# EricSteinberger/PokerRL

Hardware: AMD Instinct MI355X
Metric: CFR+ node-updates/sec on FHP public tree (higher is better)
Workload: dtype f32

## Files before the change

### include/pokerrl_hip.h

```cpp
#ifndef POKERRL_HIP_H
#define POKERRL_HIP_H

#include <stdint.h>

#ifdef __cplusplus
extern "C" {
#endif

#define PRL_MAX_BET_SIZES 96

#define PRL_OK 0
#define PRL_ERR_ARG (-1)
#define PRL_ERR_NO_DEVICE (-2)
#define PRL_ERR_HIP (-3)
#define PRL_ERR_UNSUPPORTED (-4)
#define PRL_ERR_OOM (-5)
#define PRL_ERR_STATE (-6)

typedef struct PrlRules {
    int32_t n_hole_cards;
    int32_t n_ranks;
    int32_t n_suits;
    int32_t n_cards;
    int32_t range_size;
// ... 223 lines not shown
    PRL_SF_STRAT_F64 = 4,
    PRL_SF_REGRET = 5,
    PRL_SF_AVG = 6,
    PRL_SF_AVG_F64 = 7,
    PRL_SF_AVG_SUM = 8,
    PRL_SF_BR_IDX = 9,
    PRL_SF_EXPL_HISTORY = 10,
    PRL_SF_ITER = 11,
    PRL_SF_CONSTANTS = 12,
    PRL_SF_BYTES_ALLOCATED = 13,
    PRL_SF_ENGINE = 14,
    PRL_SF_GRAPH_REPLAY = 15,
    PRL_SF_EXCHANGES = 17,
    PRL_SF_VMM_RANGES = 18,
    PRL_SF_AVG_PAIRS = 19,
    PRL_SF_EXPLICIT_STRATEGY = 16
};
int32_t prl_solver_get(prl_solver_t* solver, int32_t field, void* out);
int32_t prl_solver_set_strategy_device(prl_solver_t* solver, const prl_tree_t* tree, const float* d_probs, int32_t n_actions);
int32_t prl_solver_get_cols(prl_solver_t* solver, int32_t field, int64_t col_begin, int64_t n_cols, void* out);

int32_t prl_lbr_checkdown_equity(const PrlRules* rules, const int8_t* board_dealt, int32_t n_dealt, const int8_t* lbr_hand,
                                 const float* ranges, int32_t n_q, float* out_wp);
int32_t prl_lbr_checkdown_equity_batch(const PrlRules* rules, int32_t n_req, const int8_t* boards_dealt , const int32_t* n_dealt,
                                       const int8_t* lbr_hands , const float* ranges ,
                                       const int32_t* n_q, int32_t q_stride, float* out_wp );

int32_t prl_lbr_batch_run(const PrlGame* lbr_game, const PrlGame* agent_game, const PrlRules* rules, int32_t n_envs, int32_t agent_seat,
                          int32_t check_to_round, int32_t agent_kind, uint32_t agent_seed, uint32_t episode_base, double reward_scalar,
                          double ev_normalizer, const int8_t* cards, float* out_winnings, uint64_t* out_stats4, float* out_device_ms);
// ... 35 lines not shown
```

### pokerrl_amd/_native.py

```python
import ctypes
import os

import numpy as np

_HERE = os.path.dirname(os.path.abspath(__file__))
EXCHANGE_FN = ctypes.CFUNCTYPE(ctypes.c_int32, ctypes.c_void_p, ctypes.c_void_p, ctypes.c_void_p, ctypes.c_uint64)
LIB_PATH = os.environ.get("POKERRL_AMD_LIB", os.path.join(_HERE, "lib", "libpokerrl_hip.so"))

PRL_MAX_BET_SIZES = 96


class NativeError(RuntimeError):
    status = None


ERR_ARG, ERR_NO_DEVICE, ERR_HIP, ERR_UNSUPPORTED, ERR_OOM, ERR_STATE = -1, -2, -3, -4, -5, -6


class PrlRules(ctypes.Structure):
    _fields_ = [
        ("n_hole_cards", ctypes.c_int32), ("n_ranks", ctypes.c_int32), ("n_suits", ctypes.c_int32),
        ("n_cards", ctypes.c_int32), ("range_size", ctypes.c_int32), ("n_rounds", ctypes.c_int32),
        ("board_cards_in_round", ctypes.c_int32 * 4), ("n_board_cards", ctypes.c_int32),
        ("btn_first_postflop", ctypes.c_int32), ("rank_rule", ctypes.c_int32),
# ... 511 lines not shown
        check(self._L.prl_tree_obs_stats(self._h, _ptr(out)), self._L)
        return dict(state_bytes=int(out[0]), states_ms=float(out[1]), obs_ms=float(out[2]), obs_bytes=int(out[3]))

    def __del__(self):
        try:
            if self._h:
                self._L.prl_tree_destroy(self._h)
                self._h = None
        except Exception:
            pass


OBS_VANILLA, OBS_HISTORY, OBS_FLAT_HU_LIMIT = 0, 1, 2

SF = dict(reach=0, ev=1, ev_br=2, strategy=3, strat_f64=4, regret=5, avg=6, avg_f64=7, avg_sum=8, br_idx=9,
          expl_history=10, iter=11, constants=12, bytes_allocated=13, engine=14, graph_replay=15, explicit_strategy=16, exchanges=17, vmm_ranges=18, avg_pairs=19)
VARIANTS = {"vanilla": 0, "plus": 1, "linear": 2}
ENGINES = {"auto": 0, "levels": 1, "fused": 2}


class NativeSolver:

    def __init__(self, tree, variant, delay=0, engine="auto", _lib=None, shard=None, avg_dtype="f64", place=None, probe_iters=4, board_mult=None,
                 symmetrize=False):
        self._L = _lib or tree._L
        self.placement_ms, self.placement_chosen = None, None
        if _lib is None and self._L is lib():
            require_device()
        self.tree = tree
        self._h = ctypes.c_void_p()
        v = VARIANTS[variant] if isinstance(variant, str) else int(variant)
# ... 226 lines not shown
        finally:
            for n in names:
                qs[n].put(None)
            for t in th:
                t.join()
        return {n: h.hexdigest() for n, h in hs.items()}

    def get(self, name):
        n, c, R = self.n_nodes, self.n_cols, self.R
        shape, dtype = {
            "reach": ((n, 2, R), np.float32), "ev": ((n, 2, R), np.float32), "ev_br": ((n, 2, R), np.float32),
            "strategy": ((c, R), np.float64), "strat_f64": ((n,), np.uint8), "regret": ((c, R), np.float32),
            "avg": ((c, R), np.float64), "avg_f64": ((n,), np.uint8), "avg_sum": ((c, R), np.float32),
            "br_idx": ((n, R), np.int32), "constants": ((2,), np.float32), "bytes_allocated": ((1,), np.int64),
            "explicit_strategy": ((1,), np.int32), "exchanges": ((1,), np.int64), "vmm_ranges": ((2,), np.int64),
            "avg_pairs": ((1,), np.int64),
        }.get(name, (None, None))
        if name == "expl_history":
            shape, dtype = (self.iter + 1, 2), np.float32
        out = np.zeros(shape, dtype)
        self._call("prl_solver_get", SF[name], _ptr(out))
        return out
```

### pokerrl_amd/csrc/prl_fhp.h

```cpp
#pragma once
#include "prl_defs.h"
#include "prl_solver_types.h"
#include "prl_tree.h"

enum { PRL_SRC_REGRET = 0, PRL_SRC_UNIFORM64 = 1, PRL_SRC_ARR64 = 2, PRL_SRC_ARR32 = 3,
       PRL_SRC_STRAT32 = 4 ,
       PRL_SRC_AVGF32 = 5  };
enum { PRL_FHP_UPDATE0 = 0, PRL_FHP_UPDATE1 = 1, PRL_FHP_EVAL = 2, PRL_FHP_UPDATE0_EVAL = 3, PRL_FHP_UPDATE0_BR = 4, PRL_FHP_UPDATE1_EVAL1 = 5,
       PRL_FHP_EVAL0 = 6 };
constexpr bool prl_fhp_runs_seat(int mode, int p) {
    return mode == PRL_FHP_EVAL || mode == PRL_FHP_UPDATE0_EVAL ? true
         : (mode == PRL_FHP_UPDATE1 || mode == PRL_FHP_UPDATE1_EVAL1) ? p == 1 : p == 0;
}
constexpr bool prl_fhp_updates(int mode, int p) {
    return p == 0 ? (mode == PRL_FHP_UPDATE0 || mode == PRL_FHP_UPDATE0_EVAL || mode == PRL_FHP_UPDATE0_BR)
                  : (mode == PRL_FHP_UPDATE1 || mode == PRL_FHP_UPDATE1_EVAL1);
}
constexpr bool prl_fhp_with_br(int mode) { return mode >= PRL_FHP_EVAL; }
constexpr int prl_fhp_out_width(int mode) {
    return mode == PRL_FHP_UPDATE1_EVAL1 ? 3
         : (prl_fhp_runs_seat(mode, 0) && prl_fhp_runs_seat(mode, 1) ? 2 : 1) * (prl_fhp_with_br(mode) ? 2 : 1);
}

#define PRL_FHP_MAX_NODES 40
// ... 134 lines not shown
    int32_t np;
    int32_t variant, iter;
    int32_t max_grid;
    int32_t shape;
    int32_t n_cols_board, n_dec;
    int32_t dec_nch[PRL_FHP_MAX_DEC], dec_col0[PRL_FHP_MAX_DEC];
    float chance_prob, eq_const;
    float pot[PRL_FHP_MAX_NODES];
    const float* chance_reach;
    const float* board_w;
    float* regret;
    double* avg;
    float* avg32;
    int32_t avg_mode;
    double m_old, m_new;
    int32_t avg_pair;
    double m_old_prev, m_new_prev;
    float* avg_sum;
    int32_t avgsum_mask, avgsum_iter[2];
    int32_t block_sum;
    int32_t exp;
    int32_t no_steady;
    const double* strat_arr;
    float* board_out;
    const int16_t* plan_pp;
    const uint32_t* plan_clx;
    unsigned long long* timing;
};

int prl_fhp_match_shape(const PrlFlatTree& t, int* chance_node, int* first_board_node, int* col_base, float* pots );

int prl_launch_fhp_pass(const PrlFhpParams& prm, int mode, int src0, int src1, void* stream);
void prl_launch_fhp_strategy_from_regret(const PrlFhpParams& prm, double* out_region, void* stream);
void prl_launch_fhp_avg_from_sum(const PrlFhpParams& prm, void* stream);
void prl_launch_fhp_symmetrize(const float* in, int n_vec, int R, const int32_t* class_of, const int32_t* class_start, const int32_t* class_hands, float* out, void* stream);
void prl_launch_fhp_expand(const PrlFhpParams& prm, const void* region, int elem, int b0, int nb, const void* fill_by_col, const void* blocked_src,
                           void* dst, void* stream);
void prl_launch_fhp_compact(const PrlFhpParams& prm, const void* src, int elem, int b0, int nb, void* region, void* blocked_dst, void* stream);
#define PRL_FHP_NBLOCKED (1326 - 1081)
void prl_launch_fhp_chance_sum(const float* d_board_vals, int n_boards, int W, float* d_scratch, float* d_dest, void* stream);
int prl_fhp_units_at_level(int n_boards, int level);
void prl_launch_fhp_chance_partial(const float* d_board_vals, int n_boards, int level, int W, float* d_scratch, float* d_units, void* stream);
void prl_launch_fhp_chance_partial_from_blocks(const float* d_blocks, int n_blk, int level, int W, float* d_units, void* stream);
void prl_launch_fhp_chance_finish(const float* d_units, int n_units, int level, int W, float* d_scratch, float* d_dest, void* stream);
void prl_launch_fhp_compact_gathered(const float* d_in, int world, int n_which, int n_units, int W, float* d_out, void* stream);
```

### pokerrl_amd/csrc/prl_fhp_kernels.hip

```cpp
#include <type_traits>

#include "prl_device.h"
#include "prl_fhp.h"
#include "prl_kernels.h"


#if defined(PRL_EMU)
#define FHP_LB(t, w)
#else
#define FHP_LB(t, w) __launch_bounds__(t, w)
#endif

#define FHP_THREADS 768
#define FHP_SLOTS 2
#define FHP_LAUNCH_BOUNDS FHP_LB(768, 3)
#define FHP_SPEC PrlFhpSpec15
namespace fhp_shape15 {
#include "prl_fhp_pass.inc"
}
#undef FHP_SPEC
#define FHP_SPEC PrlFhpSpec9
namespace fhp_shape9 {
#include "prl_fhp_pass.inc"
}
#undef FHP_SPEC
#if !defined(PRL_FHP_NO_SHAPE21)
#define FHP_SPEC PrlFhpSpec21
namespace fhp_shape21 {
#include "prl_fhp_pass.inc"
}
#undef FHP_SPEC
#endif
#undef FHP_THREADS
#undef FHP_SLOTS
#undef FHP_LAUNCH_BOUNDS

const PrlFhpShapeDesc& prl_fhp_shape_desc(int shape_id) {
    static_assert(PrlFhpDerive<PrlFhpSpec15>::MAX_A <= PRL_FHP_BOARD_MAX_ACTIONS && PrlFhpDerive<PrlFhpSpec9>::MAX_A <= PRL_FHP_BOARD_MAX_ACTIONS &&
                      PrlFhpDerive<PrlFhpSpec21>::MAX_A <= PRL_FHP_BOARD_MAX_ACTIONS,
                  "the board pass and the readers of PrlFhpParams::dec_nch hold PRL_FHP_BOARD_MAX_ACTIONS actions per node");
    static const PrlFhpShapeDesc d[PRL_FHP_N_SHAPES] = {prl_fhp_describe<PrlFhpDerive<PrlFhpSpec15>>(), prl_fhp_describe<PrlFhpDerive<PrlFhpSpec9>>(),
                                                        prl_fhp_describe<PrlFhpDerive<PrlFhpSpec21>>()};
    return d[shape_id];
}

bool prl_fhp_shape_compiled(int shape_id) {
#if !defined(PRL_FHP_NO_SHAPE21)
    return shape_id >= 0 && shape_id < PRL_FHP_N_SHAPES;
#else
    return shape_id == PRL_FHP_SHAPE_15 || shape_id == PRL_FHP_SHAPE_9;
// ... 215 lines not shown
```

### pokerrl_amd/csrc/prl_fhp_pass.inc

```
#ifndef FHP_NPAD
#define FHP_NPAD 1088
#define FHP_NLIVE 1081
#define FHP_NCARDS 52
#define FHP_R 1326
#define FHP_NP PRL_FHP_NP
#define FHP_NSHOW (PrlFhpShape::N_SHOW)
#define FHP_NFOLD (PrlFhpShape::N_FOLD)
#define FHP_NVEC (PrlFhpShape::N_SHOW + PrlFhpShape::N_FOLD)
#endif
typedef PrlFhpDerive<FHP_SPEC> PrlFhpShape;
#if defined(FHP_EXPERIMENT)
#define FHP_EXP(c, bit) (((c).prm->exp & (bit)) != 0)
#define FHP_AVG_PIPELINED(c) true
#define FHP_TERMINAL_CACHE(c) true
#else
#define FHP_EXP(c, bit) false
#define FHP_AVG_PIPELINED(c) true
#define FHP_TERMINAL_CACHE(c) true
#endif
static_assert(PrlFhpShape::subtree_size(0) == PrlFhpShape::N_NODES, "the spec is one DFS pre-order tree");
static_assert(FHP_NP == FHP_NPAD && FHP_NP == PRL_PP_NPAD && FHP_R == PRL_PP_R && FHP_SLOTS == 2, "sorted storage: a column holds the padded sorted domain, a lane two positions");

#include "prl_fhp_div.inc"
struct FhpV { FhpF v; };
// ... 146 lines not shown

PRL_DEV PRL_INLINE FhpLds fhp_lds() {
    FhpLds L;
    float* f = (float*)prl_smem();
    L.y = f; f += FHP_NVEC * FHP_NPAD;
    L.K = f; f += 2 * FHP_NSHOW * FHP_NPAD;
    L.Tc = f; f += FHP_NFOLD * 64;
    L.Tt = f; f += 16;
    L.acc = f; f += FHP_ACC_WORDS;
    L.pf_rg = f; f += FHP_RG_IN_LDS ? FHP_PF_RG_WORDS : 0;
    L.pf_clx = (uint32_t*)f; f += FHP_PF_AREA(PRL_CLX_WORDS);
    L.pf_pp = (uint32_t*)f; f += FHP_PF_AREA(FHP_PP_WORDS);
    return L;
}

constexpr bool fhp_steady_plus(int steady) { return steady == 1 || steady == 4 || steady == 5 || steady == 6; }
template <int STEADY>
struct FhpCtxT {
    static constexpr bool own_after_b(int src_opp) { return src_opp == PRL_SRC_REGRET && !fhp_steady_plus(STEADY); }
    PRL_DEV PRL_INLINE int variant() const {
        if constexpr (fhp_steady_plus(STEADY)) return PRL_CFR_PLUS;
        else if constexpr (STEADY == 2) return PRL_CFR_LINEAR;
        else if constexpr (STEADY == 3) return PRL_CFR_VANILLA;
        else return variant_;
    }
    PRL_DEV PRL_INLINE bool first_iteration() const { if constexpr (STEADY != 0) return false; else return iter == 0; }
    PRL_DEV PRL_INLINE int avg_mode() const {
        if constexpr (STEADY == 1 || STEADY == 4 || STEADY == 6) return 2;
        else if constexpr (STEADY != 0) return 0;
        else return prm->avg_pair == PRL_FHP_AVG_DEFERRED ? 0 : prm->avg_mode;
    }
    PRL_DEV PRL_INLINE bool avg_catch_up() const { if constexpr (STEADY == 6) return true; else if constexpr (STEADY != 0) return false; else return prm->avg_pair == PRL_FHP_AVG_CATCH_UP; }
    PRL_DEV PRL_INLINE int avgsum_mask() const { if constexpr (fhp_steady_plus(STEADY)) return 0; else return prm->avgsum_mask; }
    PRL_DEV PRL_INLINE bool avg32() const { if constexpr (STEADY == 4) return true; else if constexpr (STEADY != 0) return false; else return prm->avg32 != nullptr; }
    FhpLds L;
    int wave;
    uint32_t pf_lds;
    uint32_t rec0, rec1;
    int p0;
    int gsm1[FHP_SLOTS];
    int gem1[FHP_SLOTS];
    bool live[FHP_SLOTS];
    int c1[FHP_SLOTS], c2[FHP_SLOTS];
    int sh[FHP_SLOTS];
    bool active;
    bool valid;
    float eq_const;
// ... 213 lines not shown
        if (lane == LAST_LANES - 1) L.Tt[v] = pj;
    };
    for (int v = wave; v < FHP_NVEC; v += n_waves) {
        if (v < 2 * FHP_NPAIRS) range_prefix(std::integral_constant<int, 2>(), v);
        else range_prefix(std::integral_constant<int, 1>(), v);
    }
    prl_dma_wait();
    FHP_SYNC(c, 3);
}

constexpr bool fhp_is_dec_of(int P, int n) { return PrlFhpShape::kind(n) == PRL_NODE_DECISION && PrlFhpShape::actor(n) == P; }
constexpr bool fhp_completes_before(int a, int b) {
    if (a > b) return a < b + PrlFhpShape::subtree_size(b);
    return !(b < a + PrlFhpShape::subtree_size(a));
}
constexpr int fhp_completion_rank(int P, int n) {
    int r = 0;
    for (int m = 0; m < PrlFhpShape::N_NODES; ++m)
        if (m != n && fhp_is_dec_of(P, m) && fhp_completes_before(m, n)) ++r;
    return r;
}
constexpr int fhp_node_of_rank(int P, int r) {
    for (int m = 0; m < PrlFhpShape::N_NODES; ++m)
        if (fhp_is_dec_of(P, m) && fhp_completion_rank(P, m) == r) return m;
    return -1;
}
template <int NODE, class C>
PRL_DEV PRL_INLINE void fhp_request_old_average(C& c) {
    if constexpr (NODE >= 0) {
        constexpr int col0 = PrlFhpShape::col0(NODE);
#pragma unroll
        for (int i = 0; i < PrlFhpShape::nch(NODE); ++i)
        {
            if (c.avg32()) {
                float f[FHP_SLOTS];
                fhp_gload_nt(c.prm->avg32 + c.cofs + (size_t)(col0 + i) * FHP_NP, f);
                for (int k = 0; k < FHP_SLOTS; ++k) c.av_old[col0 + i][k] = (double)f[k];
            } else fhp_gload_nt(c.prm->avg + c.cofs + (size_t)(col0 + i) * FHP_NP, c.av_old[col0 + i]);
        }
    }
}

template <int MODE, int P, int S0, int S1, int NODE, int TC = 0>
struct FhpUp {
    template <class C>
// ... 46 lines not shown
            for (int k = 0; k < FHP_SLOTS; ++k) {
                const float ek = c.live[k] ? e[k] : 0.f;
                ev.v[k] = ek;
                br.v[k] = ek;
            }
            if constexpr (TC == 1) {
                if constexpr (kind == PRL_NODE_TERM_SHOWDOWN) fhp_lds_store2(L.K + slot * FHP_NPAD, c.p0, ev.v);
                else { L.y[yb + ys * c.p0] = ev.v[0]; L.y[yb + ys * (c.p0 + 1)] = ev.v[1]; }
            }
        } else {
            constexpr int a = PrlFhpShape::actor(NODE);
            constexpr int A = PrlFhpShape::nch(NODE);
            constexpr int col0 = PrlFhpShape::col0(NODE);
            constexpr bool UPD = a == P && prl_fhp_updates(MODE, P);
            if constexpr (UPD) {
                if (c.avg_mode() == 2 && !FHP_AVG_PIPELINED(c)) fhp_request_old_average<NODE>(c);
            }
            FhpV ce[3], cb[3];
            FhpUp<MODE, P, S0, S1, PrlFhpShape::child(NODE, 0), TC>::run(c, R, ce[0], cb[0]);
            FhpUp<MODE, P, S0, S1, PrlFhpShape::child(NODE, 1), TC>::run(c, R, ce[1], cb[1]);
            if constexpr (A > 2) FhpUp<MODE, P, S0, S1, PrlFhpShape::child(NODE, 2), TC>::run(c, R, ce[2], cb[2]);
            if constexpr (a == P) {
                constexpr int SRC = P == 0 ? S0 : S1;
                typedef typename FhpScalar<SRC>::type S;
                S s[3][FHP_SLOTS];
                fhp_node_strategy<SRC, A, S>(c, R, col0, s);
                if constexpr (sizeof(S) == sizeof(float)) {
                    FhpF sv[3];
                    for (int i = 0; i < A; ++i)
                        for (int k = 0; k < FHP_SLOTS; ++k) sv[i][k] = (float)s[i][k];
                    FhpF acc = sv[0] * ce[0].v;
// ... 17 lines not shown
                        const FhpF d = ce[i].v - ev.v;
                        FhpF rv = d;
                        if (!c.first_iteration()) {
                            FhpF old;
                            for (int k = 0; k < FHP_SLOTS; ++k) old[k] = SRC == PRL_SRC_REGRET ? R.rg[col0 + i][k] : 0.f;
                            rv = c.variant() == PRL_CFR_LINEAR ? ((float)(c.iter + 1) * d) + old : d + old;
                        }
                        for (int k = 0; k < FHP_SLOTS; ++k) {
                            float r = rv[k];
                            if (c.variant() == PRL_CFR_PLUS) r = r > 0.f ? r : 0.f;
                            rn[i][k] = r;
                        }
                        fhp_gstore_nt(c.prm->regret + c.cofs + (size_t)(col0 + i) * FHP_NP, rn[i]);
                    }
                    constexpr bool KEEP = MODE == PRL_FHP_UPDATE1_EVAL1;
                    if (KEEP || c.avg_mode()) {
                        float t[3][FHP_SLOTS], sum[FHP_SLOTS];
                        for (int k = 0; k < FHP_SLOTS; ++k) {
                            sum[k] = 0.f;
                            for (int i = 0; i < A; ++i) {
                                t[i][k] = c.variant() == PRL_CFR_PLUS ? rn[i][k] : (rn[i][k] > 0.f ? rn[i][k] : 0.f);
                                sum[k] = sum[k] + t[i][k];
                            }
                        }
                        float qn[3][FHP_SLOTS];
#if !defined(FHP_DIV_FAST) || defined(FHP_NEWSTRAT_GENERIC)
                        fhp_regret_match<A>(t, sum, qn, false);
#else
                        fhp_regret_match<A>(t, sum, qn, prl_ballot(!fhp_node_in_box<A>(t, sum)) == 0ull);
#endif
                        for (int i = 0; i < A; ++i) {
                            double an[FHP_SLOTS];
                            for (int k = 0; k < FHP_SLOTS; ++k) {
                                const float sn = qn[i][k];
                                if (KEEP) R.rg[col0 + i][k] = sn;
                                double ao = c.av_old[col0 + i][k];
                                if constexpr (SRC == PRL_SRC_REGRET) {
                                    if (c.avg_catch_up()) ao = c.prm->m_old_prev * ao + c.prm->m_new_prev * (double)s[i][k];
                                }
                                an[k] = c.avg_mode() == 2 ? c.prm->m_old * ao + c.prm->m_new * (double)sn : (double)sn;
                            }
                            if (c.avg_mode()) {
                                if (c.avg32()) {
                                    float af[FHP_SLOTS];
                                    for (int k = 0; k < FHP_SLOTS; ++k) af[k] = (float)an[k];
                                    fhp_gstore_nt(c.prm->avg32 + c.cofs + (size_t)(col0 + i) * FHP_NP, af);
                                } else fhp_gstore_nt(c.prm->avg + c.cofs + (size_t)(col0 + i) * FHP_NP, an);
                            }
                        }
                    }
                    if (c.avg_mode() == 2 && FHP_AVG_PIPELINED(c)) fhp_request_old_average<fhp_node_of_rank(P, fhp_completion_rank(P, NODE) + 2)>(c);
                }
            } else {
                FhpF acc = ce[0].v, accb = cb[0].v;
                for (int i = 1; i < A; ++i) { acc = acc + ce[i].v; accb = accb + cb[i].v; }
                ev.v = acc;
                br.v = accb;
            }
        }
    }
};

struct FhpSrc { const float* rg; const uint32_t* clx; const int16_t* pp; };
PRL_DEV PRL_INLINE FhpSrc fhp_sources(const PrlFhpParams& prm, int b) {
    FhpSrc s;
    s.rg = prm.regret + (size_t)b * PrlFhpShape::N_COLS * FHP_NP;
// ... 62 lines not shown
    fhp_scan_phases(c, [&]() {});
    if (FIRST && next_b >= 0 && c.active) {
        const FhpSrc nsrc = fhp_sources(*c.prm, next_b);
        const uint32_t s2 = (c.L.pf_pp + fhp_lead(nsrc.pp))[prl_tid()];
#pragma unroll
        for (int k = 0; k < FHP_SLOTS; ++k) {
            const int sh = (int)((s2 >> (16 * k)) & 0xFFFFu);
            c.nr0[k] = c.prm->chance_reach[sh];
            c.nr1[k] = c.prm->chance_reach[c.prm->R + sh];
        }
    }
    if (FIRST && next_b >= 0) c.nw = c.prm->board_w[next_b];
    FHP_TICK(c, 3);
    if (c.active) {
        if constexpr (prl_fhp_updates(MODE, P)) {
            if (c.avg_mode() == 2 && FHP_AVG_PIPELINED(c)) {
                fhp_request_old_average<fhp_node_of_rank(P, 0)>(c);
                fhp_request_old_average<fhp_node_of_rank(P, 1)>(c);
            }
        }
        if constexpr (MODE == PRL_FHP_UPDATE1_EVAL1) {
            if (FHP_TERMINAL_CACHE(c)) FhpUp<MODE, P, S0, S1, 0, 1>::run(c, R, ev, br);
            else FhpUp<MODE, P, S0, S1, 0>::run(c, R, ev, br);
        } else {
            FhpUp<MODE, P, S0, S1, 0>::run(c, R, ev, br);
        }
    }
    FHP_TICK(c, 4);
}

template <int MODE, int S0, int S1, int STEADY>
FHP_LAUNCH_BOUNDS PRL_GLOBAL void prl_k_fhp_pass(PrlFhpParams prm) {
    constexpr int PF_SEAT = prl_fhp_runs_seat(MODE, 0) ? 1 : 0;
// ... 196 lines not shown
    }
    if (prm.block_sum && b_begin < b_end) {
        prl_sync_lds();
        flush_block((b_end - 1) / PRL_CHANCE_BLOCK);
    }
#ifdef PRL_FHP_TIMING
    if (tid == 0) for (int i = 0; i < 6; ++i) atomicAdd(prm.timing + i, (unsigned long long)c.t_acc[i]);
#endif
}

template <int MODE, int S0, int S1, int STEADY = 0>
static void fhp_launch_t(const PrlFhpParams& prm, int grid, void* stream) {
    PRL_LAUNCH((prl_k_fhp_pass<MODE, S0, S1, STEADY>), grid, FHP_THREADS, FHP_LDS_BYTES, stream, prm);
}

int launch_pass(const PrlFhpParams& prm, int mode, int src0, int src1, void* stream) {
    if (prm.n_boards <= 0) return PRL_OK;
    if (prm.R != FHP_R) return PRL_ERR_UNSUPPORTED;
    if (((prm.avgsum_mask & 1) && src0 != PRL_SRC_REGRET) || ((prm.avgsum_mask & 2) && src1 != PRL_SRC_REGRET)) return PRL_ERR_UNSUPPORTED;
    static_assert(FHP_NVEC <= 16 && FHP_LDS_BYTES <= 160 * 1024, "terminal vectors + prefetch area of this shape must fit the CU's LDS");
    int grid = prm.n_boards < prm.max_grid ? prm.n_boards : prm.max_grid;
    const int key = mode * 100 + src0 * 10 + src1;
    const int steady = prm.no_steady || prm.iter == 0 ? 0
                       : (prm.variant == PRL_CFR_PLUS && prm.avg_mode == 2 && prm.avgsum_mask == 0)
                           ? (prm.avg32 ? 4 : prm.avg_pair == PRL_FHP_AVG_DEFERRED ? 5 : prm.avg_pair == PRL_FHP_AVG_CATCH_UP ? 6 : 1)
                       : (prm.variant == PRL_CFR_LINEAR && prm.avg_mode == 0) ? 2
                       : (prm.variant == PRL_CFR_VANILLA && prm.avg_mode == 0) ? 3 : 0;
    switch (key) {
        case PRL_FHP_UPDATE0 * 100 + PRL_SRC_UNIFORM64 * 10 + PRL_SRC_UNIFORM64: fhp_launch_t<PRL_FHP_UPDATE0, PRL_SRC_UNIFORM64, PRL_SRC_UNIFORM64>(prm, grid, stream); break;
        case PRL_FHP_UPDATE1 * 100 + PRL_SRC_REGRET * 10 + PRL_SRC_UNIFORM64: fhp_launch_t<PRL_FHP_UPDATE1, PRL_SRC_REGRET, PRL_SRC_UNIFORM64>(prm, grid, stream); break;
        case PRL_FHP_UPDATE0 * 100 + PRL_SRC_REGRET * 10 + PRL_SRC_REGRET: fhp_launch_t<PRL_FHP_UPDATE0, PRL_SRC_REGRET, PRL_SRC_REGRET>(prm, grid, stream); break;
        case PRL_FHP_UPDATE1 * 100 + PRL_SRC_REGRET * 10 + PRL_SRC_REGRET: fhp_launch_t<PRL_FHP_UPDATE1, PRL_SRC_REGRET, PRL_SRC_REGRET>(prm, grid, stream); break;
        case PRL_FHP_UPDATE0_EVAL * 100 + PRL_SRC_REGRET * 10 + PRL_SRC_REGRET: fhp_launch_t<PRL_FHP_UPDATE0_EVAL, PRL_SRC_REGRET, PRL_SRC_REGRET>(prm, grid, stream); break;
        case PRL_FHP_UPDATE0_BR * 100 + PRL_SRC_REGRET * 10 + PRL_SRC_REGRET:
            if (steady == 1) fhp_launch_t<PRL_FHP_UPDATE0_BR, PRL_SRC_REGRET, PRL_SRC_REGRET, 1>(prm, grid, stream);
            else if (steady == 4) fhp_launch_t<PRL_FHP_UPDATE0_BR, PRL_SRC_REGRET, PRL_SRC_REGRET, 4>(prm, grid, stream);
            else if (steady == 5) fhp_launch_t<PRL_FHP_UPDATE0_BR, PRL_SRC_REGRET, PRL_SRC_REGRET, 5>(prm, grid, stream);
            else if (steady == 6) fhp_launch_t<PRL_FHP_UPDATE0_BR, PRL_SRC_REGRET, PRL_SRC_REGRET, 6>(prm, grid, stream);
            else if (steady == 2) fhp_launch_t<PRL_FHP_UPDATE0_BR, PRL_SRC_REGRET, PRL_SRC_REGRET, 2>(prm, grid, stream);
            else if (steady == 3) fhp_launch_t<PRL_FHP_UPDATE0_BR, PRL_SRC_REGRET, PRL_SRC_REGRET, 3>(prm, grid, stream);
            else fhp_launch_t<PRL_FHP_UPDATE0_BR, PRL_SRC_REGRET, PRL_SRC_REGRET>(prm, grid, stream);
            break;
        case PRL_FHP_UPDATE1_EVAL1 * 100 + PRL_SRC_REGRET * 10 + PRL_SRC_REGRET:
            if (steady == 1) fhp_launch_t<PRL_FHP_UPDATE1_EVAL1, PRL_SRC_REGRET, PRL_SRC_REGRET, 1>(prm, grid, stream);
            else if (steady == 4) fhp_launch_t<PRL_FHP_UPDATE1_EVAL1, PRL_SRC_REGRET, PRL_SRC_REGRET, 4>(prm, grid, stream);
            else if (steady == 5) fhp_launch_t<PRL_FHP_UPDATE1_EVAL1, PRL_SRC_REGRET, PRL_SRC_REGRET, 5>(prm, grid, stream);
            else if (steady == 6) fhp_launch_t<PRL_FHP_UPDATE1_EVAL1, PRL_SRC_REGRET, PRL_SRC_REGRET, 6>(prm, grid, stream);
            else if (steady == 2) fhp_launch_t<PRL_FHP_UPDATE1_EVAL1, PRL_SRC_REGRET, PRL_SRC_REGRET, 2>(prm, grid, stream);
            else if (steady == 3) fhp_launch_t<PRL_FHP_UPDATE1_EVAL1, PRL_SRC_REGRET, PRL_SRC_REGRET, 3>(prm, grid, stream);
            else fhp_launch_t<PRL_FHP_UPDATE1_EVAL1, PRL_SRC_REGRET, PRL_SRC_REGRET>(prm, grid, stream);
            break;
        case PRL_FHP_EVAL0 * 100 + PRL_SRC_REGRET * 10 + PRL_SRC_REGRET: fhp_launch_t<PRL_FHP_EVAL0, PRL_SRC_REGRET, PRL_SRC_REGRET>(prm, grid, stream); break;
        case PRL_FHP_EVAL * 100 + PRL_SRC_UNIFORM64 * 10 + PRL_SRC_UNIFORM64: fhp_launch_t<PRL_FHP_EVAL, PRL_SRC_UNIFORM64, PRL_SRC_UNIFORM64>(prm, grid, stream); break;
        case PRL_FHP_EVAL * 100 + PRL_SRC_REGRET * 10 + PRL_SRC_REGRET: fhp_launch_t<PRL_FHP_EVAL, PRL_SRC_REGRET, PRL_SRC_REGRET>(prm, grid, stream); break;
        case PRL_FHP_EVAL * 100 + PRL_SRC_ARR64 * 10 + PRL_SRC_ARR64: fhp_launch_t<PRL_FHP_EVAL, PRL_SRC_ARR64, PRL_SRC_ARR64>(prm, grid, stream); break;
        case PRL_FHP_EVAL * 100 + PRL_SRC_STRAT32 * 10 + PRL_SRC_STRAT32: fhp_launch_t<PRL_FHP_EVAL, PRL_SRC_STRAT32, PRL_SRC_STRAT32>(prm, grid, stream); break;
        case PRL_FHP_EVAL * 100 + PRL_SRC_AVGF32 * 10 + PRL_SRC_AVGF32: fhp_launch_t<PRL_FHP_EVAL, PRL_SRC_AVGF32, PRL_SRC_AVGF32>(prm, grid, stream); break;
        case PRL_FHP_EVAL * 100 + PRL_SRC_ARR32 * 10 + PRL_SRC_ARR32: fhp_launch_t<PRL_FHP_EVAL, PRL_SRC_ARR32, PRL_SRC_ARR32>(prm, grid, stream); break;
        default: return PRL_ERR_UNSUPPORTED;
    }
    return PRL_OK;
}
// ... 1 lines not shown
```

### pokerrl_amd/csrc/prl_solver.hip

```cpp
#include <math.h>
#include <stdlib.h>
#include <string.h>
#if !defined(PRL_EMU)
#include <dlfcn.h>
#include <rccl/rccl.h>
#endif

#include <algorithm>
#include <string>
#include <unordered_map>
#include <vector>

#include "prl_cards.h"
#include "prl_device.h"
#include "prl_fhp.h"
#include "prl_host.h"
#include "prl_kernels.h"
#include "prl_policy.h"
#include "prl_rt.h"
#include "prl_solver_types.h"
#include "prl_st.h"

#define PRL_NODE_LEAF 4

// ... 49 lines not shown
    int chance_trunk = -1;
    float* d_sum_scratch = nullptr;
    double* d_user_strategy = nullptr;
    float* d_user_strategy32 = nullptr;
    int user_strategy_f64 = -1;
    int src[2] = {PRL_SRC_UNIFORM64, PRL_SRC_UNIFORM64};
    bool board_avg_f64 = false;
    bool board_avg_stale = false;
    bool avg_deferred = false;
    float* d_regret = nullptr;
    double* d_avg = nullptr;
    float* d_avg32 = nullptr;
    bool avg_f32 = false;
    long long n_exchanges = 0;
    long long n_avg_pairs = 0;
    void* rccl_comm = nullptr;
    bool streets = false;
    PrlStPlanHost st;
    PrlStParams sp{};
    struct StLevelDev { PrlStInst* inst = nullptr; } st_dev[PRL_ST_MAX_GROUPS];
    struct StStreetDev { float* leaf_reach = nullptr; float* val = nullptr; } st_str[PRL_ST_MAX_LEVELS + 1];
    PrlFlatTree chain_ft;
    PrlDevTree Tc{};
    float* d_chain_ev = nullptr;
    PrlStChainTerm* d_chain_terms = nullptr;
    PrlStChainBundle* d_chain_bundles = nullptr;
    hipStream_t chain_stream = nullptr;
    hipEvent_t chain_fork = nullptr, chain_join = nullptr;
    std::vector<int32_t> chain_level_start;
    int n_chain_term = 0, n_chain_bundles = 0, n_chain = 0;
// ... 1665 lines not shown
    return do_update_reach(s, s->S);
}

int32_t prl_solver_update_reach(prl_solver_t* s) {
    if (!s) { prl_set_error("NULL solver"); return PRL_ERR_ARG; }
    s->ev_valid = false;
    return do_update_reach(s, s->S);
}

int32_t prl_solver_compute_ev(prl_solver_t* s) {
    if (!s) { prl_set_error("NULL solver"); return PRL_ERR_ARG; }
    s->ev_valid = false;
    return ensure_ev(s);
}

static int iteration_core(prl_solver* s, bool closing_eval, int avg_pair = PRL_FHP_AVG_NORMAL) {
    if (s->fused && s->user_strategy_f64 >= 0) { prl_set_error("call reset() / fill_uniform() before iterating after set_strategy()"); return PRL_ERR_STATE; }
    int mode = 0;
    double m_old = 0., m_new = 0.;
    cfr_plus_weights(s, s->iter, &mode, &m_old, &m_new);
    s->fp.avg_mode = mode;
    s->fp.m_old = m_old;
    s->fp.m_new = m_new;
    s->fp.avg_pair = avg_pair;
    s->fp.m_old_prev = s->fp.m_new_prev = 0.;
    if (avg_pair == PRL_FHP_AVG_CATCH_UP) {
        int mode_prev = 0;
        cfr_plus_weights(s, s->iter - 1, &mode_prev, &s->fp.m_old_prev, &s->fp.m_new_prev);
        if (mode_prev != 2 || mode != 2) { prl_set_error("paired average update outside the blending iterations"); return PRL_ERR_STATE; }
    }
    if (avg_pair == PRL_FHP_AVG_DEFERRED) s->avg_deferred = true;
    for (int p = 0; p < 2; ++p) {
        bool second_half = false;
        if (s->fused) {
            const bool steady = s->src[0] == PRL_SRC_REGRET && s->src[1] == PRL_SRC_REGRET;
            if (p == 0 && s->expl_pending && s->have_half) {
                TRY(expl_to_history(s));
                TRY(do_compute_ev(s, s->S, PRL_FHP_UPDATE0_BR));
                s->expl_pending = false;
                s->have_half = false;
            } else if (p == 0 && s->expl_pending) {
                TRY(expl_to_history(s));
                TRY(do_compute_ev(s, s->S, PRL_FHP_UPDATE0_EVAL));
                s->expl_pending = false;
            } else if (p == 1 && steady) {
                TRY(do_compute_ev(s, s->S, PRL_FHP_UPDATE1_EVAL1));
                second_half = true;
            } else TRY(do_compute_ev(s, s->S, p == 0 ? PRL_FHP_UPDATE0 : PRL_FHP_UPDATE1));
        } else TRY(ensure_ev(s));
        prl_launch_regret_strategy(s->T, s->S, s->d_nodes_p[p], s->n_nodes_p[p], p, s->variant, s->iter, s->stream);
        s->src[p] = PRL_SRC_REGRET;
        s->ev_valid = false;
        TRY(do_update_reach(s, s->S));
        prl_launch_average(s->T, s->S, s->d_nodes_p[p], s->n_nodes_p[p], p, s->variant, s->iter, mode, m_old, m_new, s->stream);
        if (s->fused && mode) s->board_avg_f64 = mode == 2;
        if (s->fused && s->variant != PRL_CFR_PLUS) s->avg_pending[p] = s->iter;
        if (second_half) s->have_half = true;
    }
    s->fp.avg_mode = 0;
    s->fp.avg_pair = PRL_FHP_AVG_NORMAL;
    if (avg_pair == PRL_FHP_AVG_CATCH_UP) { s->avg_deferred = false; ++s->n_avg_pairs; }
    if (s->sorted) blocked_avg_step(s, mode, m_old, m_new);
    s->iter += 1;
    if (s->fused && !closing_eval) {
        s->expl_pending = true;
        PRL_HIP_TRY(hipGetLastError());
        return PRL_OK;
    }
    if (s->fused && s->have_half) {
        TRY(do_compute_ev(s, s->S, PRL_FHP_EVAL0));
        s->have_half = false;
        s->ev_valid = true;
    } else TRY(ensure_ev(s));
    PRL_HIP_TRY(hipGetLastError());
    return record_expl(s);
}
// ... 126 lines not shown
    if (!s) { prl_set_error("NULL solver"); return PRL_ERR_ARG; }
    return prl_solver_iterations(s, 1);
}

int32_t prl_solver_iterations(prl_solver_t* s, int32_t n) {
    if (!s) { prl_set_error("NULL solver"); return PRL_ERR_ARG; }
    if (!s->fused && s->small_tree && n > 0) return small_tree_iterations(s, n);
#if !defined(PRL_EMU)
    if (!s->fused && !s->graphs_off && n > 0) {
        const int rc = levels_graph_iterations(s, n);
        if (rc != PRL_ERR_UNSUPPORTED) return rc;
    }
#endif
    if (s->avg_deferred) { prl_set_error("an iteration failed between the two halves of a paired average update; reset() or load_state()"); return PRL_ERR_STATE; }
    const bool may_pair = s->fused && !s->streets && s->variant == PRL_CFR_PLUS && !s->avg_f32 && !getenv("PRL_FHP_NO_AVG_PAIR");
    bool deferred = false;
    for (int i = 0; i < n; ++i) {
        int avg_pair = PRL_FHP_AVG_NORMAL;
        if (deferred) avg_pair = PRL_FHP_AVG_CATCH_UP;
        else if (may_pair && i + 1 < n && s->src[0] == PRL_SRC_REGRET && s->src[1] == PRL_SRC_REGRET && s->user_strategy_f64 < 0) {
            int mode; double m_old, m_new;
            cfr_plus_weights(s, s->iter, &mode, &m_old, &m_new);
            if (mode == 2) avg_pair = PRL_FHP_AVG_DEFERRED;
        }
        TRY(iteration_core(s, i == n - 1, avg_pair));
        deferred = avg_pair == PRL_FHP_AVG_DEFERRED;
    }
    return PRL_OK;
}

int32_t prl_solver_time_iterations_ex(prl_solver_t* s, int32_t n, float* out_ms, float* out_pass_ms, int32_t* out_n_pass) {
    if (!s || !out_ms || n < 0) { prl_set_error("bad argument"); return PRL_ERR_ARG; }
    hipEvent_t e0, e1;
    PRL_HIP_TRY(hipEventCreate(&e0));
    PRL_HIP_TRY(hipEventCreate(&e1));
    TRY(ensure_hist(s, s->iter + n + 1));
    s->time_passes = s->fused && out_pass_ms != nullptr;
    PRL_HIP_TRY(hipEventRecord(e0, s->stream));
    int rc = prl_solver_iterations(s, n);
    s->time_passes = false;
    if (rc == PRL_OK) {
// ... 315 lines not shown
                const size_t tcb = (size_t)s->T.n_cols * s->R;
                PRL_HIP_TRY(hipMemcpyAsync(out, s->S.avg_sum, tcb * 4, hipMemcpyDeviceToHost, s->stream));
                TRY(sorted_get_boards(s, s->S.avg_sum + s->board_ofs, 4, nullptr, nullptr, (float*)out + tcb, 4, 0, s->fp.n_boards));
                return prl_solver_sync(s);
            }
            src = s->S.avg_sum; bytes = nc * 4; break;
        case PRL_SF_BR_IDX: TRY(ensure_ev(s)); src = s->S.br_idx; bytes = (size_t)s->T.n_nodes * s->T.R * 4; break;
        case PRL_SF_EXPL_HISTORY: src = s->d_expl_hist; bytes = (size_t)(s->iter + 1) * 2 * 4; break;
        case PRL_SF_ITER: *(int32_t*)out = s->iter; return PRL_OK;
        case PRL_SF_CONSTANTS: ((float*)out)[0] = s->T.chance_prob; ((float*)out)[1] = s->T.eq_const; return PRL_OK;
        case PRL_SF_BYTES_ALLOCATED: *(int64_t*)out = (int64_t)s->bytes_allocated; return PRL_OK;
        case PRL_SF_ENGINE: *(int32_t*)out = s->fused ? PRL_ENGINE_FUSED : PRL_ENGINE_LEVELS; return PRL_OK;
        case PRL_SF_GRAPH_REPLAY: *(int32_t*)out = s->levels_graph_exec != nullptr; return PRL_OK;
        case PRL_SF_EXCHANGES: *(int64_t*)out = (int64_t)s->n_exchanges; return PRL_OK;
        case PRL_SF_AVG_PAIRS: *(int64_t*)out = (int64_t)s->n_avg_pairs; return PRL_OK;
        case PRL_SF_VMM_RANGES: {
            int64_t bytes = 0;
#if !defined(PRL_EMU)
            for (void* r : s->vmm) bytes += (int64_t)((PrlVmmRange*)r)->size;
#endif
            ((int64_t*)out)[0] = (int64_t)s->vmm.size(); ((int64_t*)out)[1] = bytes; return PRL_OK;
        }
        case PRL_SF_EXPLICIT_STRATEGY: *(int32_t*)out = s->fused ? s->user_strategy_f64 : -1; return PRL_OK;
        default: prl_set_error("unknown solver field"); return PRL_ERR_ARG;
    }
    if (!src) { prl_set_error("field not available for this variant"); return PRL_ERR_STATE; }
    const bool col_field = field == PRL_SF_STRATEGY || field == PRL_SF_REGRET || field == PRL_SF_AVG || field == PRL_SF_AVG_SUM;
    if (col_field && !s->col_dfs.empty()) {
        std::vector<char> tmp(bytes);
        PRL_HIP_TRY(hipMemcpyAsync(tmp.data(), src, bytes, hipMemcpyDeviceToHost, s->stream));
// ... 287 lines not shown
```

Measured before the change: 193.2 million.

## Split paired average updates into two staggered column sets across iterations

```diff
diff --git a/include/pokerrl_hip.h b/include/pokerrl_hip.h
--- a/include/pokerrl_hip.h
+++ b/include/pokerrl_hip.h
@@ -261,6 +261,7 @@
     PRL_SF_EXCHANGES = 17,
     PRL_SF_VMM_RANGES = 18,
     PRL_SF_AVG_PAIRS = 19,
+    PRL_SF_AVG_SPLIT_PAIRS = 20,
     PRL_SF_EXPLICIT_STRATEGY = 16
 };
 int32_t prl_solver_get(prl_solver_t* solver, int32_t field, void* out);
diff --git a/pokerrl_amd/_native.py b/pokerrl_amd/_native.py
--- a/pokerrl_amd/_native.py
+++ b/pokerrl_amd/_native.py
@@ -549,7 +549,7 @@
 OBS_VANILLA, OBS_HISTORY, OBS_FLAT_HU_LIMIT = 0, 1, 2
 
 SF = dict(reach=0, ev=1, ev_br=2, strategy=3, strat_f64=4, regret=5, avg=6, avg_f64=7, avg_sum=8, br_idx=9,
-          expl_history=10, iter=11, constants=12, bytes_allocated=13, engine=14, graph_replay=15, explicit_strategy=16, exchanges=17, vmm_ranges=18, avg_pairs=19)
+          expl_history=10, iter=11, constants=12, bytes_allocated=13, engine=14, graph_replay=15, explicit_strategy=16, exchanges=17, vmm_ranges=18, avg_pairs=19, avg_split_pairs=20)
 VARIANTS = {"vanilla": 0, "plus": 1, "linear": 2}
 ENGINES = {"auto": 0, "levels": 1, "fused": 2}
 
@@ -806,7 +806,7 @@
             "avg": ((c, R), np.float64), "avg_f64": ((n,), np.uint8), "avg_sum": ((c, R), np.float32),
             "br_idx": ((n, R), np.int32), "constants": ((2,), np.float32), "bytes_allocated": ((1,), np.int64),
             "explicit_strategy": ((1,), np.int32), "exchanges": ((1,), np.int64), "vmm_ranges": ((2,), np.int64),
-            "avg_pairs": ((1,), np.int64),
+            "avg_pairs": ((1,), np.int64), "avg_split_pairs": ((1,), np.int64),
         }.get(name, (None, None))
         if name == "expl_history":
             shape, dtype = (self.iter + 1, 2), np.float32
diff --git a/pokerrl_amd/csrc/prl_fhp.h b/pokerrl_amd/csrc/prl_fhp.h
--- a/pokerrl_amd/csrc/prl_fhp.h
+++ b/pokerrl_amd/csrc/prl_fhp.h
@@ -172,7 +172,7 @@
     float* avg32;
     int32_t avg_mode;
     double m_old, m_new;
-    int32_t avg_pair;
+    int32_t avg_pair, avg_pair_b;
     double m_old_prev, m_new_prev;
     float* avg_sum;
     int32_t avgsum_mask, avgsum_iter[2];
@@ -189,6 +189,7 @@
 int prl_fhp_match_shape(const PrlFlatTree& t, int* chance_node, int* first_board_node, int* col_base, float* pots );
 
 int prl_launch_fhp_pass(const PrlFhpParams& prm, int mode, int src0, int src1, void* stream);
+bool prl_fhp_avg_split_supported(int shape_id);
 void prl_launch_fhp_strategy_from_regret(const PrlFhpParams& prm, double* out_region, void* stream);
 void prl_launch_fhp_avg_from_sum(const PrlFhpParams& prm, void* stream);
 void prl_launch_fhp_symmetrize(const float* in, int n_vec, int R, const int32_t* class_of, const int32_t* class_start, const int32_t* class_hands, float* out, void* stream);
diff --git a/pokerrl_amd/csrc/prl_fhp_kernels.hip b/pokerrl_amd/csrc/prl_fhp_kernels.hip
--- a/pokerrl_amd/csrc/prl_fhp_kernels.hip
+++ b/pokerrl_amd/csrc/prl_fhp_kernels.hip
@@ -14,6 +14,7 @@
 #define FHP_THREADS 768
 #define FHP_SLOTS 2
 #define FHP_LAUNCH_BOUNDS FHP_LB(768, 3)
+#define FHP_AVG_SPLIT 1
 #define FHP_SPEC PrlFhpSpec15
 namespace fhp_shape15 {
 #include "prl_fhp_pass.inc"
@@ -25,6 +26,8 @@
 }
 #undef FHP_SPEC
 #if !defined(PRL_FHP_NO_SHAPE21)
+#undef FHP_AVG_SPLIT
+#define FHP_AVG_SPLIT 0
 #define FHP_SPEC PrlFhpSpec21
 namespace fhp_shape21 {
 #include "prl_fhp_pass.inc"
@@ -34,6 +37,9 @@
 #undef FHP_THREADS
 #undef FHP_SLOTS
 #undef FHP_LAUNCH_BOUNDS
+#undef FHP_AVG_SPLIT
+
+bool prl_fhp_avg_split_supported(int shape_id) { return shape_id == PRL_FHP_SHAPE_15 || shape_id == PRL_FHP_SHAPE_9; }
 
 const PrlFhpShapeDesc& prl_fhp_shape_desc(int shape_id) {
     static_assert(PrlFhpDerive<PrlFhpSpec15>::MAX_A <= PRL_FHP_BOARD_MAX_ACTIONS && PrlFhpDerive<PrlFhpSpec9>::MAX_A <= PRL_FHP_BOARD_MAX_ACTIONS &&
diff --git a/pokerrl_amd/csrc/prl_fhp_pass.inc b/pokerrl_amd/csrc/prl_fhp_pass.inc
--- a/pokerrl_amd/csrc/prl_fhp_pass.inc
+++ b/pokerrl_amd/csrc/prl_fhp_pass.inc
@@ -184,9 +184,33 @@
     return L;
 }
 
-constexpr bool fhp_steady_plus(int steady) { return steady == 1 || steady == 4 || steady == 5 || steady == 6; }
+constexpr int FHP_STEADY_PAIR0 = 16;
+constexpr int fhp_kind_code(int k) { return k == 1 ? 0 : k == 5 ? 1 : 2; }
+constexpr int fhp_steady_pair(int ka, int kb) { return ka == kb ? ka : FHP_STEADY_PAIR0 + 4 * fhp_kind_code(ka) + fhp_kind_code(kb); }
+constexpr int fhp_code_kind(int c) { return c == 0 ? 1 : c == 1 ? 5 : 6; }
+constexpr int fhp_set_kind(int steady, int set) {
+    return steady < FHP_STEADY_PAIR0 ? steady : fhp_code_kind(set == 0 ? (steady - FHP_STEADY_PAIR0) / 4 : (steady - FHP_STEADY_PAIR0) % 4);
+}
+constexpr bool fhp_steady_plus(int steady) { return steady == 1 || steady == 4 || steady == 5 || steady == 6 || steady >= FHP_STEADY_PAIR0; }
+constexpr int fhp_avg_set(int n) {
+    int cols[2] = {0, 0};
+    for (int a = PrlFhpShape::MAX_A; a >= 1; --a)
+        for (int m = 0; m < PrlFhpShape::N_NODES; ++m)
+            if (PrlFhpShape::kind(m) == PRL_NODE_DECISION && PrlFhpShape::actor(m) == PrlFhpShape::actor(n) && PrlFhpShape::nch(m) == a) {
+                const int set = cols[1] <= cols[0] ? 1 : 0;
+                if (m == n) return set;
+                cols[set] += a;
+            }
+    return 0;
+}
+constexpr bool fhp_may_load_avg(int steady, int n) {
+    if (steady == 0) return true;
+    const int k = fhp_set_kind(steady, fhp_avg_set(n));
+    return k == 1 || k == 4 || k == 6;
+}
 template <int STEADY>
 struct FhpCtxT {
+    static constexpr int steady = STEADY;
     static constexpr bool own_after_b(int src_opp) { return src_opp == PRL_SRC_REGRET && !fhp_steady_plus(STEADY); }
     PRL_DEV PRL_INLINE int variant() const {
         if constexpr (fhp_steady_plus(STEADY)) return PRL_CFR_PLUS;
@@ -195,12 +219,18 @@
         else return variant_;
     }
     PRL_DEV PRL_INLINE bool first_iteration() const { if constexpr (STEADY != 0) return false; else return iter == 0; }
+    template <int NODE>
     PRL_DEV PRL_INLINE int avg_mode() const {
-        if constexpr (STEADY == 1 || STEADY == 4 || STEADY == 6) return 2;
-        else if constexpr (STEADY != 0) return 0;
-        else return prm->avg_pair == PRL_FHP_AVG_DEFERRED ? 0 : prm->avg_mode;
-    }
-    PRL_DEV PRL_INLINE bool avg_catch_up() const { if constexpr (STEADY == 6) return true; else if constexpr (STEADY != 0) return false; else return prm->avg_pair == PRL_FHP_AVG_CATCH_UP; }
+        constexpr int set = fhp_avg_set(NODE);
+        if constexpr (STEADY == 0) return (set == 0 ? prm->avg_pair : prm->avg_pair_b) == PRL_FHP_AVG_DEFERRED ? 0 : prm->avg_mode;
+        else return fhp_may_load_avg(STEADY, NODE) ? 2 : 0;
+    }
+    template <int NODE>
+    PRL_DEV PRL_INLINE bool avg_catch_up() const {
+        constexpr int set = fhp_avg_set(NODE);
+        if constexpr (STEADY == 0) return (set == 0 ? prm->avg_pair : prm->avg_pair_b) == PRL_FHP_AVG_CATCH_UP;
+        else return fhp_set_kind(STEADY, set) == 6;
+    }
     PRL_DEV PRL_INLINE int avgsum_mask() const { if constexpr (fhp_steady_plus(STEADY)) return 0; else return prm->avgsum_mask; }
     PRL_DEV PRL_INLINE bool avg32() const { if constexpr (STEADY == 4) return true; else if constexpr (STEADY != 0) return false; else return prm->avg32 != nullptr; }
     FhpLds L;
@@ -444,21 +474,22 @@
     if (a > b) return a < b + PrlFhpShape::subtree_size(b);
     return !(b < a + PrlFhpShape::subtree_size(a));
 }
-constexpr int fhp_completion_rank(int P, int n) {
+constexpr int fhp_completion_rank(int steady, int P, int n) {
     int r = 0;
     for (int m = 0; m < PrlFhpShape::N_NODES; ++m)
-        if (m != n && fhp_is_dec_of(P, m) && fhp_completes_before(m, n)) ++r;
+        if (m != n && fhp_is_dec_of(P, m) && fhp_may_load_avg(steady, m) && fhp_completes_before(m, n)) ++r;
     return r;
 }
-constexpr int fhp_node_of_rank(int P, int r) {
+constexpr int fhp_node_of_rank(int steady, int P, int r) {
     for (int m = 0; m < PrlFhpShape::N_NODES; ++m)
-        if (fhp_is_dec_of(P, m) && fhp_completion_rank(P, m) == r) return m;
+        if (fhp_is_dec_of(P, m) && fhp_may_load_avg(steady, m) && fhp_completion_rank(steady, P, m) == r) return m;
     return -1;
 }
 template <int NODE, class C>
 PRL_DEV PRL_INLINE void fhp_request_old_average(C& c) {
     if constexpr (NODE >= 0) {
         constexpr int col0 = PrlFhpShape::col0(NODE);
+        if (c.template avg_mode<NODE>() == 2)
 #pragma unroll
         for (int i = 0; i < PrlFhpShape::nch(NODE); ++i)
         {
@@ -535,7 +566,7 @@
             constexpr int col0 = PrlFhpShape::col0(NODE);
             constexpr bool UPD = a == P && prl_fhp_updates(MODE, P);
             if constexpr (UPD) {
-                if (c.avg_mode() == 2 && !FHP_AVG_PIPELINED(c)) fhp_request_old_average<NODE>(c);
+                if (!FHP_AVG_PIPELINED(c)) fhp_request_old_average<NODE>(c);
             }
             FhpV ce[3], cb[3];
             FhpUp<MODE, P, S0, S1, PrlFhpShape::child(NODE, 0), TC>::run(c, R, ce[0], cb[0]);
@@ -583,7 +614,8 @@
                         fhp_gstore_nt(c.prm->regret + c.cofs + (size_t)(col0 + i) * FHP_NP, rn[i]);
                     }
                     constexpr bool KEEP = MODE == PRL_FHP_UPDATE1_EVAL1;
-                    if (KEEP || c.avg_mode()) {
+                    const int avg_mode = c.template avg_mode<NODE>();
+                    if (KEEP || avg_mode) {
                         float t[3][FHP_SLOTS], sum[FHP_SLOTS];
                         for (int k = 0; k < FHP_SLOTS; ++k) {
                             sum[k] = 0.f;
@@ -605,11 +637,11 @@
                                 if (KEEP) R.rg[col0 + i][k] = sn;
                                 double ao = c.av_old[col0 + i][k];
                                 if constexpr (SRC == PRL_SRC_REGRET) {
-                                    if (c.avg_catch_up()) ao = c.prm->m_old_prev * ao + c.prm->m_new_prev * (double)s[i][k];
+                                    if (c.template avg_catch_up<NODE>()) ao = c.prm->m_old_prev * ao + c.prm->m_new_prev * (double)s[i][k];
                                 }
-                                an[k] = c.avg_mode() == 2 ? c.prm->m_old * ao + c.prm->m_new * (double)sn : (double)sn;
+                                an[k] = avg_mode == 2 ? c.prm->m_old * ao + c.prm->m_new * (double)sn : (double)sn;
                             }
-                            if (c.avg_mode()) {
+                            if (avg_mode) {
                                 if (c.avg32()) {
                                     float af[FHP_SLOTS];
                                     for (int k = 0; k < FHP_SLOTS; ++k) af[k] = (float)an[k];
@@ -618,7 +650,9 @@
                             }
                         }
                     }
-                    if (c.avg_mode() == 2 && FHP_AVG_PIPELINED(c)) fhp_request_old_average<fhp_node_of_rank(P, fhp_completion_rank(P, NODE) + 2)>(c);
+                    if constexpr (fhp_may_load_avg(C::steady, NODE)) {
+                        if (FHP_AVG_PIPELINED(c)) fhp_request_old_average<fhp_node_of_rank(C::steady, P, fhp_completion_rank(C::steady, P, NODE) + 2)>(c);
+                    }
                 }
             } else {
                 FhpF acc = ce[0].v, accb = cb[0].v;
@@ -711,9 +745,9 @@
     FHP_TICK(c, 3);
     if (c.active) {
         if constexpr (prl_fhp_updates(MODE, P)) {
-            if (c.avg_mode() == 2 && FHP_AVG_PIPELINED(c)) {
-                fhp_request_old_average<fhp_node_of_rank(P, 0)>(c);
-                fhp_request_old_average<fhp_node_of_rank(P, 1)>(c);
+            if (FHP_AVG_PIPELINED(c)) {
+                fhp_request_old_average<fhp_node_of_rank(C::steady, P, 0)>(c);
+                fhp_request_old_average<fhp_node_of_rank(C::steady, P, 1)>(c);
             }
         }
         if constexpr (MODE == PRL_FHP_UPDATE1_EVAL1) {
@@ -940,6 +974,12 @@
     PRL_LAUNCH((prl_k_fhp_pass<MODE, S0, S1, STEADY>), grid, FHP_THREADS, FHP_LDS_BYTES, stream, prm);
 }
 
+template <int MODE, int STEADY>
+static void fhp_launch_split_t(const PrlFhpParams& prm, int grid, void* stream) {
+    if constexpr (FHP_AVG_SPLIT) fhp_launch_t<MODE, PRL_SRC_REGRET, PRL_SRC_REGRET, STEADY>(prm, grid, stream);
+    else fhp_launch_t<MODE, PRL_SRC_REGRET, PRL_SRC_REGRET>(prm, grid, stream);
+}
+
 int launch_pass(const PrlFhpParams& prm, int mode, int src0, int src1, void* stream) {
     if (prm.n_boards <= 0) return PRL_OK;
     if (prm.R != FHP_R) return PRL_ERR_UNSUPPORTED;
@@ -947,9 +987,10 @@
     static_assert(FHP_NVEC <= 16 && FHP_LDS_BYTES <= 160 * 1024, "terminal vectors + prefetch area of this shape must fit the CU's LDS");
     int grid = prm.n_boards < prm.max_grid ? prm.n_boards : prm.max_grid;
     const int key = mode * 100 + src0 * 10 + src1;
+    auto kind_of = [](int pair) { return pair == PRL_FHP_AVG_DEFERRED ? 5 : pair == PRL_FHP_AVG_CATCH_UP ? 6 : 1; };
     const int steady = prm.no_steady || prm.iter == 0 ? 0
                        : (prm.variant == PRL_CFR_PLUS && prm.avg_mode == 2 && prm.avgsum_mask == 0)
-                           ? (prm.avg32 ? 4 : prm.avg_pair == PRL_FHP_AVG_DEFERRED ? 5 : prm.avg_pair == PRL_FHP_AVG_CATCH_UP ? 6 : 1)
+                           ? (prm.avg32 ? 4 : fhp_steady_pair(kind_of(prm.avg_pair), kind_of(prm.avg_pair_b)))
                        : (prm.variant == PRL_CFR_LINEAR && prm.avg_mode == 0) ? 2
                        : (prm.variant == PRL_CFR_VANILLA && prm.avg_mode == 0) ? 3 : 0;
     switch (key) {
@@ -963,6 +1004,11 @@
             else if (steady == 4) fhp_launch_t<PRL_FHP_UPDATE0_BR, PRL_SRC_REGRET, PRL_SRC_REGRET, 4>(prm, grid, stream);
             else if (steady == 5) fhp_launch_t<PRL_FHP_UPDATE0_BR, PRL_SRC_REGRET, PRL_SRC_REGRET, 5>(prm, grid, stream);
             else if (steady == 6) fhp_launch_t<PRL_FHP_UPDATE0_BR, PRL_SRC_REGRET, PRL_SRC_REGRET, 6>(prm, grid, stream);
+            else if (steady == fhp_steady_pair(5, 1)) fhp_launch_split_t<PRL_FHP_UPDATE0_BR, fhp_steady_pair(5, 1)>(prm, grid, stream);
+            else if (steady == fhp_steady_pair(6, 5)) fhp_launch_split_t<PRL_FHP_UPDATE0_BR, fhp_steady_pair(6, 5)>(prm, grid, stream);
+            else if (steady == fhp_steady_pair(5, 6)) fhp_launch_split_t<PRL_FHP_UPDATE0_BR, fhp_steady_pair(5, 6)>(prm, grid, stream);
+            else if (steady == fhp_steady_pair(6, 1)) fhp_launch_split_t<PRL_FHP_UPDATE0_BR, fhp_steady_pair(6, 1)>(prm, grid, stream);
+            else if (steady == fhp_steady_pair(1, 6)) fhp_launch_split_t<PRL_FHP_UPDATE0_BR, fhp_steady_pair(1, 6)>(prm, grid, stream);
             else if (steady == 2) fhp_launch_t<PRL_FHP_UPDATE0_BR, PRL_SRC_REGRET, PRL_SRC_REGRET, 2>(prm, grid, stream);
             else if (steady == 3) fhp_launch_t<PRL_FHP_UPDATE0_BR, PRL_SRC_REGRET, PRL_SRC_REGRET, 3>(prm, grid, stream);
             else fhp_launch_t<PRL_FHP_UPDATE0_BR, PRL_SRC_REGRET, PRL_SRC_REGRET>(prm, grid, stream);
@@ -972,6 +1018,11 @@
             else if (steady == 4) fhp_launch_t<PRL_FHP_UPDATE1_EVAL1, PRL_SRC_REGRET, PRL_SRC_REGRET, 4>(prm, grid, stream);
             else if (steady == 5) fhp_launch_t<PRL_FHP_UPDATE1_EVAL1, PRL_SRC_REGRET, PRL_SRC_REGRET, 5>(prm, grid, stream);
             else if (steady == 6) fhp_launch_t<PRL_FHP_UPDATE1_EVAL1, PRL_SRC_REGRET, PRL_SRC_REGRET, 6>(prm, grid, stream);
+            else if (steady == fhp_steady_pair(5, 1)) fhp_launch_split_t<PRL_FHP_UPDATE1_EVAL1, fhp_steady_pair(5, 1)>(prm, grid, stream);
+            else if (steady == fhp_steady_pair(6, 5)) fhp_launch_split_t<PRL_FHP_UPDATE1_EVAL1, fhp_steady_pair(6, 5)>(prm, grid, stream);
+            else if (steady == fhp_steady_pair(5, 6)) fhp_launch_split_t<PRL_FHP_UPDATE1_EVAL1, fhp_steady_pair(5, 6)>(prm, grid, stream);
+            else if (steady == fhp_steady_pair(6, 1)) fhp_launch_split_t<PRL_FHP_UPDATE1_EVAL1, fhp_steady_pair(6, 1)>(prm, grid, stream);
+            else if (steady == fhp_steady_pair(1, 6)) fhp_launch_split_t<PRL_FHP_UPDATE1_EVAL1, fhp_steady_pair(1, 6)>(prm, grid, stream);
             else if (steady == 2) fhp_launch_t<PRL_FHP_UPDATE1_EVAL1, PRL_SRC_REGRET, PRL_SRC_REGRET, 2>(prm, grid, stream);
             else if (steady == 3) fhp_launch_t<PRL_FHP_UPDATE1_EVAL1, PRL_SRC_REGRET, PRL_SRC_REGRET, 3>(prm, grid, stream);
             else fhp_launch_t<PRL_FHP_UPDATE1_EVAL1, PRL_SRC_REGRET, PRL_SRC_REGRET>(prm, grid, stream);
diff --git a/pokerrl_amd/csrc/prl_solver.hip b/pokerrl_amd/csrc/prl_solver.hip
--- a/pokerrl_amd/csrc/prl_solver.hip
+++ b/pokerrl_amd/csrc/prl_solver.hip
@@ -87,6 +87,7 @@
     bool avg_f32 = false;
     long long n_exchanges = 0;
     long long n_avg_pairs = 0;
+    long long n_avg_split_pairs = 0;
     void* rccl_comm = nullptr;
     bool streets = false;
     PrlStPlanHost st;
@@ -1782,7 +1783,7 @@
     return ensure_ev(s);
 }
 
-static int iteration_core(prl_solver* s, bool closing_eval, int avg_pair = PRL_FHP_AVG_NORMAL) {
+static int iteration_core(prl_solver* s, bool closing_eval, int avg_pair = PRL_FHP_AVG_NORMAL, int avg_pair_b = -1) {
     if (s->fused && s->user_strategy_f64 >= 0) { prl_set_error("call reset() / fill_uniform() before iterating after set_strategy()"); return PRL_ERR_STATE; }
     int mode = 0;
     double m_old = 0., m_new = 0.;
@@ -1790,14 +1791,18 @@
     s->fp.avg_mode = mode;
     s->fp.m_old = m_old;
     s->fp.m_new = m_new;
+    const bool split = avg_pair_b >= 0 && avg_pair_b != avg_pair;
+    if (avg_pair_b < 0) avg_pair_b = avg_pair;
     s->fp.avg_pair = avg_pair;
+    s->fp.avg_pair_b = avg_pair_b;
     s->fp.m_old_prev = s->fp.m_new_prev = 0.;
-    if (avg_pair == PRL_FHP_AVG_CATCH_UP) {
+    if (avg_pair == PRL_FHP_AVG_CATCH_UP || avg_pair_b == PRL_FHP_AVG_CATCH_UP) {
         int mode_prev = 0;
         cfr_plus_weights(s, s->iter - 1, &mode_prev, &s->fp.m_old_prev, &s->fp.m_new_prev);
         if (mode_prev != 2 || mode != 2) { prl_set_error("paired average update outside the blending iterations"); return PRL_ERR_STATE; }
     }
-    if (avg_pair == PRL_FHP_AVG_DEFERRED) s->avg_deferred = true;
+    const bool defers = avg_pair == PRL_FHP_AVG_DEFERRED || avg_pair_b == PRL_FHP_AVG_DEFERRED;
+    if (defers) s->avg_deferred = true;
     for (int p = 0; p < 2; ++p) {
         bool second_half = false;
         if (s->fused) {
@@ -1826,8 +1831,10 @@
         if (second_half) s->have_half = true;
     }
     s->fp.avg_mode = 0;
-    s->fp.avg_pair = PRL_FHP_AVG_NORMAL;
-    if (avg_pair == PRL_FHP_AVG_CATCH_UP) { s->avg_deferred = false; ++s->n_avg_pairs; }
+    s->fp.avg_pair = s->fp.avg_pair_b = PRL_FHP_AVG_NORMAL;
+    s->avg_deferred = defers;
+    if (avg_pair == PRL_FHP_AVG_CATCH_UP) ++s->n_avg_pairs;
+    if (split && avg_pair_b == PRL_FHP_AVG_CATCH_UP) ++s->n_avg_split_pairs;
     if (s->sorted) blocked_avg_step(s, mode, m_old, m_new);
     s->iter += 1;
     if (s->fused && !closing_eval) {
@@ -1984,17 +1991,22 @@
 #endif
     if (s->avg_deferred) { prl_set_error("an iteration failed between the two halves of a paired average update; reset() or load_state()"); return PRL_ERR_STATE; }
     const bool may_pair = s->fused && !s->streets && s->variant == PRL_CFR_PLUS && !s->avg_f32 && !getenv("PRL_FHP_NO_AVG_PAIR");
-    bool deferred = false;
+    const bool may_split = may_pair && prl_fhp_avg_split_supported(s->fp.shape) && !getenv("PRL_FHP_NO_AVG_SPLIT");
+    int r = -1;
     for (int i = 0; i < n; ++i) {
-        int avg_pair = PRL_FHP_AVG_NORMAL;
-        if (deferred) avg_pair = PRL_FHP_AVG_CATCH_UP;
+        if (r >= 0) ++r;
         else if (may_pair && i + 1 < n && s->src[0] == PRL_SRC_REGRET && s->src[1] == PRL_SRC_REGRET && s->user_strategy_f64 < 0) {
             int mode; double m_old, m_new;
             cfr_plus_weights(s, s->iter, &mode, &m_old, &m_new);
-            if (mode == 2) avg_pair = PRL_FHP_AVG_DEFERRED;
-        }
-        TRY(iteration_core(s, i == n - 1, avg_pair));
-        deferred = avg_pair == PRL_FHP_AVG_DEFERRED;
+            if (mode == 2) r = 0;
+        }
+        const bool last = i == n - 1;
+        int avg_pair = PRL_FHP_AVG_NORMAL, avg_pair_b = -1;
+        if (r >= 0) {
+            avg_pair = r % 2 ? PRL_FHP_AVG_CATCH_UP : last ? PRL_FHP_AVG_NORMAL : PRL_FHP_AVG_DEFERRED;
+            if (may_split) avg_pair_b = r == 0 ? PRL_FHP_AVG_NORMAL : r % 2 ? (last ? PRL_FHP_AVG_NORMAL : PRL_FHP_AVG_DEFERRED) : PRL_FHP_AVG_CATCH_UP;
+        }
+        TRY(iteration_core(s, last, avg_pair, avg_pair_b));
     }
     return PRL_OK;
 }
@@ -2340,6 +2352,7 @@
         case PRL_SF_GRAPH_REPLAY: *(int32_t*)out = s->levels_graph_exec != nullptr; return PRL_OK;
         case PRL_SF_EXCHANGES: *(int64_t*)out = (int64_t)s->n_exchanges; return PRL_OK;
         case PRL_SF_AVG_PAIRS: *(int64_t*)out = (int64_t)s->n_avg_pairs; return PRL_OK;
+        case PRL_SF_AVG_SPLIT_PAIRS: *(int64_t*)out = (int64_t)s->n_avg_split_pairs; return PRL_OK;
         case PRL_SF_VMM_RANGES: {
             int64_t bytes = 0;
 #if !defined(PRL_EMU)
```

New measurement: 202.1 million (median of 6 runs). 4.6% higher.
